# VITA-Group/FasterSeg

Measured on AMD Instinct MI355X. Metric: supernet train-step images/sec @1024x2048 (1/2/4/8 GPU) + student fps, higher is better.
Workload: dtype bf16; 1 GPU; C2 student fps (BASELINE configs[1]): searched arch_1 (eval build, branches 1/32+1/16) inference 1x3x1024x2048, 19 classes, fp32 logits at input resolution; parallelism=replicas x1 (inference does not shard: no collective)

## Files before the change

### fasterseg_amd/_lib.py

```python
import ctypes
import os

_HERE = os.path.dirname(os.path.abspath(__file__))
LIB_PATH = os.path.join(_HERE, "libfasterseg_hip.so")

EXPECTED_ABI = 218
FS_F32, FS_BF16 = 0, 1
FS_CONV_RELU, FS_CONV_TRANSPOSED, FS_CONV_ACCUM, FS_CONV_RELU_TAIL = 1, 2, 4, 8
FS_CONV_KSPLIT, FS_CONV_NO_KSPLIT, FS_CONV_KSPLIT16 = 0x4000, 0x8000, 0x14000

c_int, c_ll, c_float, c_vp = ctypes.c_int, ctypes.c_longlong, ctypes.c_float, ctypes.c_void_p


class ConvDesc(ctypes.Structure):
    _fields_ = [(n, c_int) for n in ("N", "H", "W", "Cin", "Cout", "R", "S", "stride", "pad", "Ho", "Wo",
                                     "x_cs", "y_cs", "dtype", "flags", "w_os", "w_ts", "vr_H", "vr_W", "vr_relu", "bn_groups",
                                     "n_seg", "n_jump", "k_seg", "k_jump", "g_jump")]


class ZoomDesc(ctypes.Structure):
    _fields_ = [(n, c_int) for n in ("N", "H", "W", "Cin", "Cmid", "Cout", "h", "w", "Ho", "Wo", "x_cs", "y_cs", "dtype", "down", "up")]


class LogitsDesc(ctypes.Structure):
    _fields_ = [(n, c_int) for n in ("N", "h", "w", "C", "cs", "H", "W", "dtype")]


class ResizeDesc(ctypes.Structure):
    _fields_ = [(n, c_int) for n in ("N", "Hi", "Wi", "Ho", "Wo", "C", "x_cs", "y_cs", "dtype", "relu", "out_nchw")]


class EvalWindowDesc(ctypes.Structure):
    _fields_ = [(n, c_int) for n in ("H", "W", "rows", "cols", "top", "left", "oy", "ox", "crop_h", "crop_w", "pad_mode", "flip")] + [
        ("mean", c_float * 3), ("std", c_float * 3)]


class TrainSample(ctypes.Structure):
    _fields_ = [(n, c_int) for n in ("H", "W", "mirror", "sh", "sw", "pos_h", "pos_w", "top", "left", "rows", "cols", "ylin", "xlin",
                                     "ynn", "xnn", "reserved")]
# ... 98 lines not shown
    "fs_nchw_to_nhwc": [c_vp, c_int, c_int, c_int, c_int, c_vp, c_vp, c_int, c_int, c_int],
    "fs_nhwc_to_nchw": [c_vp, c_int, c_int, c_int, c_int, c_vp, c_int, c_int, c_vp],
    "fs_copy_channels": [c_vp, c_ll, c_int, c_vp, c_int, c_vp, c_int, c_int],
    "fs_axpy_channels": [c_vp, c_ll, c_int, c_vp, c_int, c_vp, c_vp, c_int, c_int, c_int],
    "fs_dot": [c_vp, c_ll, c_int, c_vp, c_int, c_vp, c_int, c_int, c_vp],
    "fs_weighted_sum": [c_vp, c_ll, c_int, c_int, c_vp, c_vp, c_vp, c_vp, c_int, c_int],
    "fs_weighted_sum_bwd": [c_vp, c_ll, c_int, c_int, c_vp, c_int, c_vp, c_vp, c_vp, c_int],
    "fs_weighted_sum_dots": [c_vp, c_ll, c_int, c_int, c_vp, c_int, c_vp, c_vp, c_int, c_vp],
    "fs_ohem_ce_fwd": [c_vp, c_vp, c_vp, c_ll, c_int, c_ll, c_int, c_vp, c_vp, c_vp],
    "fs_ohem_ce_bwd": [c_vp, c_vp, c_vp, c_vp, c_vp, c_vp, c_ll, c_int, c_ll, c_vp],
    "fs_ohem_ce_bwd_coef": [c_vp, c_vp, c_vp, c_vp, c_vp, c_vp, c_ll, c_int, c_ll, c_vp],
    "fs_ohem_select": [c_vp, c_vp, c_vp, c_vp, c_ll, c_int, c_int, c_vp, c_float, c_ll, c_vp, c_vp, c_vp, c_vp, c_ll],
    "fs_kl_distill_fwd": [c_vp, c_vp, c_vp, c_ll, c_int, c_ll, c_vp, c_vp, c_vp],
    "fs_ohem_ce_up_fwd": [c_vp, ctypes.POINTER(LogitsDesc), c_vp, c_vp, c_int, c_vp, c_vp, c_vp],
    "fs_ohem_ce_up_bwd": [c_vp, ctypes.POINTER(LogitsDesc), c_vp, c_vp, c_vp, c_vp, c_vp, c_vp, c_vp, c_ll],
    "fs_ohem_ce_up_bwd_coef": [c_vp, ctypes.POINTER(LogitsDesc), c_vp, c_vp, c_vp, c_vp, c_vp, c_vp, c_vp, c_ll],
    "fs_kl_distill_up_fwd": [c_vp, ctypes.POINTER(LogitsDesc), c_vp, ctypes.POINTER(LogitsDesc), c_vp, c_vp, c_vp, c_vp],
    "fs_kl_distill_up_bwd": [c_vp, ctypes.POINTER(LogitsDesc), c_vp, ctypes.POINTER(LogitsDesc), c_vp, c_vp, c_vp, c_vp, c_vp, c_vp,
                             c_ll],
    "fs_kl_distill_bwd": [c_vp, c_vp, c_vp, c_vp, c_vp, c_vp, c_ll, c_int, c_ll, c_vp],
    "fs_exec_program": [c_vp, c_vp, c_ll, c_vp, c_vp, c_int],
    "fs_exec_program_streams": [c_vp, c_int, c_vp, c_ll, c_vp, c_vp, c_int],
    "fs_exec_program_group": [c_vp, c_int, c_vp, c_vp, c_vp, c_vp, c_int],
    "fs_sgd_momentum_multi": [c_vp, c_vp, c_vp, c_int, c_vp, c_vp, c_vp, c_vp, c_float, c_float, c_float, c_int, c_int],
    "fs_refresh_weights": [c_vp, c_vp, c_int, c_vp, c_int],
}
_SPECIAL = {
    "fs_last_error": ([], ctypes.c_char_p),
    "fs_version": ([], c_int),
    "fs_struct_size": ([c_int], c_int),
    "fs_packed_weight_elems": ([c_int, c_int, c_int, c_int], c_ll),
    "fs_debug_force_conv_cfg": ([c_int], None),
    "fs_debug_stem_mfma": ([c_int], None),
    "fs_packed_weight_frag_elems": ([c_int, c_int, c_int], c_ll),
    "fs_sgd_chunk_elems": ([], c_int),
    "fs_sgd_tensor_chunks": ([c_ll, c_int, c_int, c_int], c_ll),
    "fs_refresh_chunk_elems": ([], c_int),
    "fs_refresh_entry_chunks": ([ctypes.POINTER(RefreshEntry)], c_ll),
    "fs_loss_up_workspace_bytes": ([ctypes.POINTER(LogitsDesc)], c_ll),
    "fs_ohem_select_workspace_bytes": ([c_ll], c_ll),
    "fs_train_batch_args_bytes": ([c_int], c_ll),
    "fs_zoom_cell_supported": ([ctypes.POINTER(ZoomDesc)], c_int),
    "fs_workspace_counter_bytes": ([], c_ll),
    "fs_set_deterministic": ([c_int], None),
    "fs_get_deterministic": ([], c_int),
    "fs_set_fp32_split": ([c_int], None),
    "fs_get_fp32_split": ([], c_int),
    "fs_census_enable": ([c_int], None),
    "fs_census_read": ([c_vp, c_int], c_int),
    "fs_census_read_kernels": ([c_vp, c_int], c_int),
    "fs_census_tag": ([c_int], None),
    "fs_census_read_tags": ([c_int, c_vp, c_vp], c_int),
    "fs_event_create": ([], c_vp),
    "fs_event_destroy": ([c_vp], None),
}
ALL_SYMBOLS = sorted(list(SIGNATURES) + list(_SPECIAL))

_lib = None


class FasterSegHipError(RuntimeError):
    pass


def lib():
    global _lib
# ... 39 lines not shown
```

### fasterseg_amd/csrc/resize.hip

```cpp
#include "common.h"
#include "group.h"

namespace fs {

static inline float host_scale(int in, int out) { return out > 1 ? (float)(in - 1) / (float)(out - 1) : 0.f; }

struct ResizeArgs {
    int N; DivInt Hi, Wi, Ho, Wo, cv; float rh, rw; const void* a; int a_cs; const void* b; int b_cs; void* out; int out_cs; int relu;
};

template <typename T>
__device__ __forceinline__ void bilinear_fwd_body(const ResizeArgs& q, int bx, int gx) {
    constexpr int VEC = Elem<T>::VEC;
    const int N = q.N, Hi = q.Hi, Wi = q.Wi, Ho = q.Ho, Wo = q.Wo, cv = q.cv, x_cs = q.a_cs, y_cs = q.out_cs, relu = q.relu;
    const float rh = q.rh, rw = q.rw;
    const T* __restrict__ x = (const T*)q.a;
    T* __restrict__ y = (T*)q.out;
    const long long total = (long long)N * Ho * Wo * cv;
    for (long long idx = bx * (long long)blockDim.x + threadIdx.x; idx < total; idx += (long long)gx * blockDim.x) {
        long long t = idx, u = fast_div(t, q.cv);
        const int c = (int)(t - u * cv) * VEC; t = u; u = fast_div(t, q.Wo);
        const int ow = (int)(t - u * Wo); t = u; u = fast_div(t, q.Ho);
        const int oh = (int)(t - u * Ho);
        const int n = (int)u;
        const Tap th = make_tap(rh, oh, Hi), tw = make_tap(rw, ow, Wi);
        const T* base = x + (long long)n * Hi * Wi * x_cs + c;
        float p00[VEC], p01[VEC], p10[VEC], p11[VEC];
        Elem<T>::unpack(ldg16(base + ((long long)th.i0 * Wi + tw.i0) * x_cs), p00);
        Elem<T>::unpack(ldg16(base + ((long long)th.i0 * Wi + tw.i1) * x_cs), p01);
        Elem<T>::unpack(ldg16(base + ((long long)th.i1 * Wi + tw.i0) * x_cs), p10);
        Elem<T>::unpack(ldg16(base + ((long long)th.i1 * Wi + tw.i1) * x_cs), p11);
#pragma unroll
        for (int i = 0; i < VEC; ++i) {
            float o = th.l0 * (tw.l0 * p00[i] + tw.l1 * p01[i]) + th.l1 * (tw.l0 * p10[i] + tw.l1 * p11[i]);
            p00[i] = relu ? fmaxf(o, 0.f) : o;
        }
        stg16(y + (((long long)n * Ho + oh) * Wo + ow) * y_cs + c, Elem<T>::pack(p00));
    }
}

template <typename T> struct Quad;
template <> struct Quad<float> {
    static __device__ __forceinline__ void load(const float* p, float* o) {
        const f32x4 v = *reinterpret_cast<const f32x4*>(p);
        o[0] = v[0]; o[1] = v[1]; o[2] = v[2]; o[3] = v[3];
    }
};
template <> struct Quad<bf16_t> {
    static __device__ __forceinline__ void load(const bf16_t* p, float* o) {
        const uint2 v = *reinterpret_cast<const uint2*>(p);
        o[0] = __uint_as_float(v.x << 16); o[1] = __uint_as_float(v.x & 0xffff0000u);
        o[2] = __uint_as_float(v.y << 16); o[3] = __uint_as_float(v.y & 0xffff0000u);
    }
};
template <typename TO> __device__ __forceinline__ void store4(TO* dst, const float* v);
template <> __device__ __forceinline__ void store4<float>(float* dst, const float* v) {
    __builtin_nontemporal_store(f32x4{v[0], v[1], v[2], v[3]}, reinterpret_cast<f32x4*>(dst));
}
template <> __device__ __forceinline__ void store4<bf16_t>(bf16_t* dst, const float* v) {
    uint2 o;
    o.x = (uint32_t)f32_to_bf16(v[0]) | ((uint32_t)f32_to_bf16(v[1]) << 16);
    o.y = (uint32_t)f32_to_bf16(v[2]) | ((uint32_t)f32_to_bf16(v[3]) << 16);
    *reinterpret_cast<uint2*>(dst) = o;
}

template <typename T, typename TO>
__global__ __launch_bounds__(256) void bilinear_fwd_nchw_kernel(int N, int Hi, int Wi, int Ho, int Wo, int C, float rh, float rw,
                                                                const T* __restrict__ x, int x_cs, TO* __restrict__ y) {
    const int wq = Wo >> 2;
    const int cg = (C + 3) >> 2;
    const long long total = (long long)N * cg * Ho * wq;
    for (long long idx = blockIdx.x * (long long)blockDim.x + threadIdx.x; idx < total;
         idx += (long long)gridDim.x * blockDim.x) {
        long long t = idx;
        const int ow0 = divmod32(t, wq) * 4;
        const int oh = divmod32(t, Ho);
        const int c0 = divmod32(t, cg) * 4;
        const int n = (int)t;
        const Tap th = make_tap(rh, oh, Hi);
        const T* r0 = x + ((long long)n * Hi + th.i0) * Wi * x_cs + c0;
        const T* r1 = x + ((long long)n * Hi + th.i1) * Wi * x_cs + c0;
        float out[4][4];
#pragma unroll
        for (int q = 0; q < 4; ++q) {
            const Tap tw = make_tap(rw, ow0 + q, Wi);
            float p00[4], p01[4], p10[4], p11[4];
            Quad<T>::load(r0 + (long long)tw.i0 * x_cs, p00);
            Quad<T>::load(r0 + (long long)tw.i1 * x_cs, p01);
            Quad<T>::load(r1 + (long long)tw.i0 * x_cs, p10);
            Quad<T>::load(r1 + (long long)tw.i1 * x_cs, p11);
#pragma unroll
            for (int k = 0; k < 4; ++k)
                out[k][q] = th.l0 * (tw.l0 * p00[k] + tw.l1 * p01[k]) + th.l1 * (tw.l0 * p10[k] + tw.l1 * p11[k]);
        }
#pragma unroll
        for (int k = 0; k < 4; ++k)
            if (c0 + k < C) store4<TO>(y + (((long long)n * C + c0 + k) * Ho + oh) * Wo + ow0, out[k]);
    }
}

template <typename T, typename TO>
__global__ void bilinear_fwd_nchw_scalar_kernel(int N, int Hi, int Wi, int Ho, int Wo, int C, float rh, float rw,
                                                const T* __restrict__ x, int x_cs, TO* __restrict__ y) {
    const long long total = (long long)N * C * Ho * Wo;
    for (long long idx = blockIdx.x * (long long)blockDim.x + threadIdx.x; idx < total;
         idx += (long long)gridDim.x * blockDim.x) {
        long long t = idx;
        const int ow = divmod32(t, Wo);
        const int oh = divmod32(t, Ho);
        const int c = divmod32(t, C);
        const int n = (int)t;
        const Tap th = make_tap(rh, oh, Hi), tw = make_tap(rw, ow, Wi);
        const T* b = x + (long long)n * Hi * Wi * x_cs + c;
        const float p00 = Elem<T>::load(b + ((long long)th.i0 * Wi + tw.i0) * x_cs);
        const float p01 = Elem<T>::load(b + ((long long)th.i0 * Wi + tw.i1) * x_cs);
        const float p10 = Elem<T>::load(b + ((long long)th.i1 * Wi + tw.i0) * x_cs);
        const float p11 = Elem<T>::load(b + ((long long)th.i1 * Wi + tw.i1) * x_cs);
        Elem<TO>::store(y + idx, th.l0 * (tw.l0 * p00 + tw.l1 * p01) + th.l1 * (tw.l0 * p10 + tw.l1 * p11));
    }
}

__device__ __forceinline__ void cand_range(float scale, int i, int out_size, int& lo, int& hi) {
    if (scale <= 0.f) {
        lo = 0;
        hi = out_size - 1;
        return;
    }
    const float inv = 1.f / scale;
    lo = (int)floorf((float)(i - 1) * inv) - 1;
    hi = (int)ceilf((float)(i + 1) * inv) + 1;
    if (lo < 0) lo = 0;
    if (hi > out_size - 1) hi = out_size - 1;
}
__device__ __forceinline__ float tap_weight(const Tap& t, int i) {
    float w = 0.f;
    if (t.i0 == i) w += t.l0;
    if (t.i1 == i) w += t.l1;
    return w;
}

constexpr int BWD_TAPS = 6;

template <typename T>
__device__ __forceinline__ void bilinear_bwd_body(const ResizeArgs& q, int bx, int gx) {
    constexpr int VEC = Elem<T>::VEC;
// ... 163 lines not shown
        const int ih = divmod32(t, Hi);
        const int c = divmod32(t, C);
        const int n = (int)t;
        int lo, hi;
        cand_range(rh, ih, Ho, lo, hi);
        const float* plane = tmp + ((long long)n * C + c) * Ho * Wi + iw;
        float acc = 0.f;
        for (int o0 = lo; o0 <= hi; o0 += 8) {
            float v[8];
#pragma unroll
            for (int u = 0; u < 8; ++u) v[u] = plane[(long long)min(o0 + u, Ho - 1) * Wi];
#pragma unroll
            for (int u = 0; u < 8; ++u) {
                const int oh = o0 + u;
                const float w = (oh <= hi) ? tap_weight(make_tap(rh, oh, Hi), ih) : 0.f;
                acc += w * v[u];
            }
        }
        Elem<T>::store(dx + (((long long)n * Hi + ih) * Wi + iw) * dx_cs + c, acc);
    }
}

static inline int grid_for(long long work, int block = 256, int cap = 16384) {
    long long g = (work + block - 1) / block;
    if (g < 1) g = 1;
    if (g > cap) g = cap;
    return (int)g;
}

}

using namespace fs;

static fs_status check_resize(const char* fn, const fs_resize_desc* d) {
    FS_REQUIRE(d, FS_ERR_INVALID, "%s: null descriptor", fn);
    FS_REQUIRE(d->N > 0 && d->Hi > 0 && d->Wi > 0 && d->Ho > 0 && d->Wo > 0 && d->C > 0, FS_ERR_INVALID,
               "%s: non-positive dimension", fn);
    FS_REQUIRE(d->dtype == FS_F32 || d->dtype == FS_BF16, FS_ERR_INVALID, "%s: bad dtype", fn);
    if (!d->out_nchw) {
        const int vec = vec_elems(d->dtype);
        FS_REQUIRE(d->C % vec == 0 && d->x_cs % vec == 0 && d->y_cs % vec == 0 && d->x_cs >= d->C && d->y_cs >= d->C,
                   FS_ERR_UNSUPPORTED, "%s: C=%d / strides (%d,%d) must be multiples of %d", fn, d->C, d->x_cs, d->y_cs, vec);
    } else {
        FS_REQUIRE(d->x_cs >= ((d->C + 3) / 4) * 4 && d->x_cs % 4 == 0, FS_ERR_INVALID,
                   "%s: NCHW output needs the input channel stride padded to a multiple of 4 (got %d for C=%d)", fn, d->x_cs,
                   d->C);
        FS_REQUIRE(!d->relu, FS_ERR_UNSUPPORTED, "%s: relu not supported with NCHW output", fn);
    }
    return FS_OK;
}

extern "C" fs_status fs_bilinear_fwd(void* stream, const fs_resize_desc* d, const void* x, void* y) {
    fs_status s = check_resize("fs_bilinear_fwd", d);
    if (s != FS_OK) return s;
    FS_REQUIRE(x && y, FS_ERR_INVALID, "fs_bilinear_fwd: null pointer");
    const float rh = host_scale(d->Hi, d->Ho), rw = host_scale(d->Wi, d->Wo);
    hipStream_t st = (hipStream_t)stream;
    FS_REQUIRE(aligned16(x) && aligned16(y), FS_ERR_INVALID, "fs_bilinear_fwd: operands must be 16-byte aligned");
    if (!d->out_nchw) {
        const int cv = d->C / vec_elems(d->dtype);
        const long long total = (long long)d->N * d->Ho * d->Wo * cv;
        const ResizeArgs q{d->N, d->Hi, d->Wi, d->Ho, d->Wo, cv, rh, rw, x, d->x_cs, nullptr, 0, y, d->y_cs, d->relu};
        FS_NOTE_BYTES((double)d->N * d->C * elem_size(d->dtype) * ((double)d->Hi * d->Wi + (double)d->Ho * d->Wo));
        if (d->dtype == FS_F32) FS_LAUNCH((bilinear_fwd_kernel<float>), dim3(grid_for(total)), dim3(256), 0, st, q);
        else FS_LAUNCH((bilinear_fwd_kernel<bf16_t>), dim3(grid_for(total)), dim3(256), 0, st, q);
    } else {
        const bool out_f32 = (d->out_nchw == 1) || d->dtype == FS_F32;
        if (d->Wo % 4 == 0) {
            const long long total = (long long)d->N * ((d->C + 3) / 4) * d->Ho * (d->Wo / 4);
            const dim3 g(grid_for(total));
            if (d->dtype == FS_F32)
                FS_LAUNCH((bilinear_fwd_nchw_kernel<float, float>), g, dim3(256), 0, st, d->N, d->Hi, d->Wi, d->Ho, d->Wo,
                                   d->C, rh, rw, (const float*)x, d->x_cs, (float*)y);
            else if (out_f32)
                FS_LAUNCH((bilinear_fwd_nchw_kernel<bf16_t, float>), g, dim3(256), 0, st, d->N, d->Hi, d->Wi, d->Ho, d->Wo,
                                   d->C, rh, rw, (const bf16_t*)x, d->x_cs, (float*)y);
            else
                FS_LAUNCH((bilinear_fwd_nchw_kernel<bf16_t, bf16_t>), g, dim3(256), 0, st, d->N, d->Hi, d->Wi, d->Ho,
                                   d->Wo, d->C, rh, rw, (const bf16_t*)x, d->x_cs, (bf16_t*)y);
        } else {
            const long long total = (long long)d->N * d->C * d->Ho * d->Wo;
            const dim3 g(grid_for(total));
            if (d->dtype == FS_F32)
                FS_LAUNCH((bilinear_fwd_nchw_scalar_kernel<float, float>), g, dim3(256), 0, st, d->N, d->Hi, d->Wi, d->Ho,
                                   d->Wo, d->C, rh, rw, (const float*)x, d->x_cs, (float*)y);
            else if (out_f32)
                FS_LAUNCH((bilinear_fwd_nchw_scalar_kernel<bf16_t, float>), g, dim3(256), 0, st, d->N, d->Hi, d->Wi, d->Ho,
                                   d->Wo, d->C, rh, rw, (const bf16_t*)x, d->x_cs, (float*)y);
            else
                FS_LAUNCH((bilinear_fwd_nchw_scalar_kernel<bf16_t, bf16_t>), g, dim3(256), 0, st, d->N, d->Hi, d->Wi,
                                   d->Ho, d->Wo, d->C, rh, rw, (const bf16_t*)x, d->x_cs, (bf16_t*)y);
        }
    }
    return check_launch("fs_bilinear_fwd");
}

extern "C" fs_status fs_bilinear_bwd_nchw(void* stream, const fs_resize_desc* d, const float* dy, float* workspace, void* dx) {
    fs_status s = check_resize("fs_bilinear_bwd_nchw", d);
    if (s != FS_OK) return s;
    FS_REQUIRE(d->out_nchw == 1, FS_ERR_INVALID, "fs_bilinear_bwd_nchw: descriptor must have out_nchw = 1");
    FS_REQUIRE(dy && workspace && dx, FS_ERR_INVALID, "fs_bilinear_bwd_nchw: null pointer");
// ... 86 lines not shown
```

### fasterseg_amd/csrc/stem.hip

```cpp
#include "common.h"

namespace fs {

template <typename T>
__global__ __launch_bounds__(256) void stem_conv_kernel(int N, int H, int W, int Ho, int Wo, int Cout,
                                                        const float* __restrict__ x, const float* __restrict__ w,
                                                        const float* __restrict__ scale, const float* __restrict__ shift,
                                                        T* __restrict__ y, int y_cs, int relu) {
    const int co0 = blockIdx.y * 16;
    const long long total = (long long)N * Ho * Wo;
    for (long long pix = blockIdx.x * (long long)blockDim.x + threadIdx.x; pix < total;
         pix += (long long)gridDim.x * blockDim.x) {
        const int ow = (int)(pix % Wo);
        const int oh = (int)((pix / Wo) % Ho);
        const int n = (int)(pix / ((long long)Wo * Ho));
        float in[27];
#pragma unroll
        for (int c = 0; c < 3; ++c)
#pragma unroll
            for (int r = 0; r < 3; ++r)
#pragma unroll
                for (int s = 0; s < 3; ++s) {
                    const int ih = oh * 2 - 1 + r, iw = ow * 2 - 1 + s;
                    const bool ok = (unsigned)ih < (unsigned)H && (unsigned)iw < (unsigned)W;
// ... 84 lines not shown
        T* dst = y + pix * y_cs + co0;
        if (co0 + 16 <= Cout) {
#pragma unroll
            for (int v = 0; v < 16 / VEC; ++v) stg16(dst + v * VEC, Elem<T>::pack(out + v * VEC));
        } else {
            for (int k = 0; k < 16 && co0 + k < Cout; ++k) Elem<T>::store(dst + k, out[k]);
        }
    }
}




struct StemTapOff {
    int off[2][2][8];
};

__host__ __device__ constexpr int stem_tap_offset(int k) {
    return k >= 27 ? -1
                   : ((((k / 3) % 3 == 1) ? 0 : 1) * 3 + (k % 3)) * (S_ROWS * S_PITCH) + ((k / 3) / 3) * S_PITCH + (((k / 3) % 3 == 0) ? 1 : 2);
}

__device__ __forceinline__ void split_bf16(const float (&v)[8], u32x4& hi, u32x4& lo) {
#pragma unroll
    for (int i = 0; i < 4; ++i) {
        const float a = v[2 * i], b = v[2 * i + 1];
        const uint32_t h = pack2_bf16(a, b);
        const float ra = a - __uint_as_float(h << 16), rb = b - __uint_as_float(h & 0xffff0000u);
        hi[i] = h;
        lo[i] = pack2_bf16(ra, rb);
    }
}

__global__ __launch_bounds__(256) void stem_mfma_kernel(int H, int W, int Ho, int Wo, int Cout, const float* __restrict__ x,
                                                        const float* __restrict__ w, const float* __restrict__ scale,
                                                        const float* __restrict__ shift, bf16_t* __restrict__ y, int y_cs, int relu) {
    constexpr int WIN = 2 * 3 * S_ROWS * S_PITCH;
    constexpr int OUT_PITCH = 32 * 2 + 16;
    __shared__ __attribute__((aligned(16))) float win[WIN + 4];
    __shared__ __attribute__((aligned(16))) unsigned char sout[4][32 * OUT_PITCH];
    const int tid = threadIdx.x, lane = tid & 63, wave = tid >> 6, l31 = lane & 31, half = lane >> 5;
    const int ow0 = blockIdx.x * S_TW, oh0 = blockIdx.y * S_TH, n = blockIdx.z;
    constexpr int VPR = S_HALF / 2;
    for (int v = tid; v < 3 * S_ROWS * VPR; v += 256) {
        const int c = v / (S_ROWS * VPR);
        const int rem = v - c * (S_ROWS * VPR);
        const int r = rem / VPR, q = rem - r * VPR;
        const int ih = 2 * oh0 - 1 + r, iw = 2 * ow0 - 4 + 4 * q;
        f32x4 t = {0.f, 0.f, 0.f, 0.f};
        if ((unsigned)ih < (unsigned)H && iw >= 0 && iw + 3 < W)
            t = *reinterpret_cast<const f32x4*>(x + (((long long)n * 3 + c) * H + ih) * W + iw);
        float* ev = win + ((0 * 3 + c) * S_ROWS + r) * S_PITCH;
        float* od = win + ((1 * 3 + c) * S_ROWS + r) * S_PITCH;
        ev[2 * q] = t[0]; od[2 * q] = t[1];
        ev[2 * q + 1] = t[2]; od[2 * q + 1] = t[3];
    }
    if (tid < 4) win[WIN + tid] = 0.f;
    const int ntiles = (Cout + 31) / 32;
    u32x4 bh[2][2], bl[2][2];
#pragma unroll
    for (int t = 0; t < 2; ++t)
#pragma unroll
        for (int kk = 0; kk < 2; ++kk) {
            float wv[8];
            const int co = t * 32 + l31;
#pragma unroll
            for (int e = 0; e < 8; ++e) {
                const int k = kk * 16 + half * 8 + e;
                wv[e] = (t < ntiles && co < Cout && k < 27) ? w[co * 27 + k] : 0.f;
            }
            split_bf16(wv, bh[t][kk], bl[t][kk]);
        }
    __syncthreads();
    const int ty = wave;
    const int oh = oh0 + ty;
    unsigned char* so = sout[wave];
#pragma unroll
    for (int h = 0; h < 2; ++h) {
        const int tx = 32 * h + l31;
        const float* base = win + (2 * ty) * S_PITCH + tx;
        u32x4 ah[2], al[2];
#pragma unroll
        for (int kk = 0; kk < 2; ++kk) {
            float av[8];
#pragma unroll
            for (int e = 0; e < 8; ++e) {
                constexpr int dummy = 0;
                (void)dummy;
                const int o0 = stem_tap_offset(kk * 16 + e), o1 = stem_tap_offset(kk * 16 + 8 + e);
                const float* p0 = o0 >= 0 ? base + o0 : win + WIN;
                const float* p1 = o1 >= 0 ? base + o1 : win + WIN;
                av[e] = *(half ? p1 : p0);
            }
            split_bf16(av, ah[kk], al[kk]);
        }
#pragma unroll
        for (int t = 0; t < 2; ++t) {
            if (t >= ntiles) break;
            f32x16 acc;
#pragma unroll
            for (int r = 0; r < 16; ++r) acc[r] = 0.f;
#pragma unroll
            for (int kk = 0; kk < 2; ++kk) {
                acc = __builtin_amdgcn_mfma_f32_32x32x16_bf16(__builtin_bit_cast(bf16x8, al[kk]), __builtin_bit_cast(bf16x8, bh[t][kk]), acc, 0, 0, 0);
                acc = __builtin_amdgcn_mfma_f32_32x32x16_bf16(__builtin_bit_cast(bf16x8, ah[kk]), __builtin_bit_cast(bf16x8, bl[t][kk]), acc, 0, 0, 0);
                acc = __builtin_amdgcn_mfma_f32_32x32x16_bf16(__builtin_bit_cast(bf16x8, ah[kk]), __builtin_bit_cast(bf16x8, bh[t][kk]), acc, 0, 0, 0);
            }
            const int co = t * 32 + l31;
            const bool cvalid = co < Cout;
            const float sc = (scale && cvalid) ? scale[co] : 1.f, sh = (shift && cvalid) ? shift[co] : 0.f;
#pragma unroll
            for (int r = 0; r < 16; ++r) {
                const int prow = (r & 3) + 8 * (r >> 2) + 4 * half;
                float o = acc[r] * sc + sh;
                if (relu) o = fmaxf(o, 0.f);
                *reinterpret_cast<bf16_t*>(so + prow * OUT_PITCH + l31 * 2) = f32_to_bf16(o);
            }
            __builtin_amdgcn_wave_barrier();
            const int cbase = t * 32;
            const int nvalid = Cout - cbase < 32 ? Cout - cbase : 32;
#pragma unroll
            for (int ps = 0; ps < 2; ++ps) {
                const int prow = ps * 16 + (lane >> 2), seg = lane & 3;
                const int ow = ow0 + 32 * h + prow;
                if (oh < Ho && ow < Wo && seg * 8 < nvalid)
                    stg16(y + (((long long)n * Ho + oh) * Wo + ow) * y_cs + cbase + seg * 8,
                          *reinterpret_cast<const u32x4*>(so + prow * OUT_PITCH + seg * 16));
            }
            __builtin_amdgcn_wave_barrier();
        }
    }
}

}

using namespace fs;

static int g_stem_mfma = 1;
extern "C" void fs_debug_stem_mfma(int on) { g_stem_mfma = on; }

extern "C" fs_status fs_conv_stem_fwd(void* stream, int N, int H, int W, int Cout, const float* x, const float* w,
                                      const float* scale, const float* shift, void* y, int y_cs, int dtype, int relu) {
    FS_REQUIRE(x && w && y, FS_ERR_INVALID, "fs_conv_stem_fwd: null pointer");
    FS_REQUIRE(N > 0 && H > 1 && W > 1 && Cout > 0, FS_ERR_INVALID, "fs_conv_stem_fwd: bad shape");
    FS_REQUIRE(dtype == FS_F32 || dtype == FS_BF16, FS_ERR_INVALID, "fs_conv_stem_fwd: bad dtype");
    FS_REQUIRE(y_cs >= Cout && y_cs % vec_elems(dtype) == 0 && aligned16(y), FS_ERR_INVALID,
               "fs_conv_stem_fwd: output slice misaligned (y_cs=%d)", y_cs);
    const int Ho = (H + 2 - 3) / 2 + 1, Wo = (W + 2 - 3) / 2 + 1;
    if (W % 4 == 0 && aligned16(x) && N <= 65535) {
        dim3 tiles((unsigned)((Wo + S_TW - 1) / S_TW), (unsigned)((Ho + S_TH - 1) / S_TH), (unsigned)N);
        if (dtype == FS_BF16 && Cout <= 64 && Cout % 8 == 0 && g_stem_mfma) {
            FS_LAUNCH(stem_mfma_kernel, tiles, dim3(256), 0, (hipStream_t)stream, H, W, Ho, Wo, Cout, x, w, scale, shift,
                               (bf16_t*)y, y_cs, relu);
            return check_launch("fs_conv_stem_fwd");
        }
        if (dtype == FS_F32)
            FS_LAUNCH((stem_lds_kernel<float>), tiles, dim3(256), 0, (hipStream_t)stream, H, W, Ho, Wo, Cout, x, w, scale,
                               shift, (float*)y, y_cs, relu);
        else
            FS_LAUNCH((stem_lds_kernel<bf16_t>), tiles, dim3(256), 0, (hipStream_t)stream, H, W, Ho, Wo, Cout, x, w, scale,
                               shift, (bf16_t*)y, y_cs, relu);
        return check_launch("fs_conv_stem_fwd");
    }
    const long long total = (long long)N * Ho * Wo;
    long long gx = (total + 255) / 256;
    if (gx > 32768) gx = 32768;
    dim3 grid((unsigned)gx, (Cout + 15) / 16);
    if (dtype == FS_F32)
        FS_LAUNCH((stem_conv_kernel<float>), grid, dim3(256), 0, (hipStream_t)stream, N, H, W, Ho, Wo, Cout, x, w, scale,
                           shift, (float*)y, y_cs, relu);
    else
        FS_LAUNCH((stem_conv_kernel<bf16_t>), grid, dim3(256), 0, (hipStream_t)stream, N, H, W, Ho, Wo, Cout, x, w, scale,
                           shift, (bf16_t*)y, y_cs, relu);
    return check_launch("fs_conv_stem_fwd");
}
```

### include/fasterseg_hip.h

```cpp
#ifndef FASTERSEG_HIP_H
#define FASTERSEG_HIP_H

#ifdef __cplusplus
extern "C" {
#endif

typedef enum { FS_OK = 0, FS_ERR_INVALID = 1, FS_ERR_UNSUPPORTED = 2, FS_ERR_LAUNCH = 3 } fs_status;
typedef enum { FS_F32 = 0, FS_BF16 = 1 } fs_dtype;

#define FS_CONV_RELU        1
#define FS_CONV_TRANSPOSED  2
#define FS_CONV_ACCUM       4
#define FS_CONV_RELU_TAIL   8
#define FS_CONV_TILE_32     0x1000
#define FS_CONV_TILE_64     0x2000
#define FS_CONV_TILE_128    0x3000
#define FS_CONV_TILE_MASK   0x3000
#define FS_CONV_KSPLIT      0x4000
#define FS_CONV_NO_KSPLIT   0x8000
#define FS_CONV_KSPLIT16    0x14000

typedef struct fs_conv_desc {
    int N, H, W, Cin;
    int Cout, R, S;
    int stride, pad;
    int Ho, Wo;
    int x_cs, y_cs;
    int dtype;
    int flags;
    int w_os, w_ts;
    int vr_H, vr_W;
    int vr_relu;
    int bn_groups;
    int n_seg, n_jump;
    int k_seg, k_jump;
    int g_jump;
} fs_conv_desc;

typedef struct fs_resize_desc {
    int N, Hi, Wi, Ho, Wo, C;
    int x_cs, y_cs;
    int dtype;
    int relu;
    int out_nchw;
} fs_resize_desc;

const char* fs_last_error(void);
#define FS_ABI_VERSION 218
int fs_version(void);
void fs_set_deterministic(int on);
int fs_get_deterministic(void);
void fs_set_fp32_split(int on);
int fs_get_fp32_split(void);
int fs_struct_size(int which);
void fs_debug_force_conv_cfg(int cfg);
long long fs_packed_weight_elems(int Cout, int R, int S, int Cin);

fs_status fs_pack_weight(void* stream, const float* w_oihw, long long o_stride, long long i_stride,
                         int Cout, int Cin, int R, int S, int dtype, int transpose_flip, void* w_packed);
fs_status fs_unpack_weight_grad(void* stream, const float* dw_packed, int Cout, int Cin, int R, int S,
                                float* dw_oihw, long long o_stride, long long i_stride, int accumulate);

fs_status fs_conv2d_fwd(void* stream, const fs_conv_desc* d, const void* x, const void* w_packed,
                        const float* scale, const float* shift, void* y, float* stats);
#define FS_CONV_WORKSPACE_BYTES (16ll << 20)
fs_status fs_conv2d_fwd_ws(void* stream, const fs_conv_desc* d, const void* x, const void* w_packed,
                           const float* scale, const float* shift, void* y, float* stats, void* workspace,
                           long long workspace_bytes);

fs_status fs_factorized_reduce_fwd(void* stream, const fs_conv_desc* d1, const void* x1, const void* w1_packed, void* y1, float* stats1,
                                   const fs_conv_desc* d2, const void* x2, const void* w2_packed, void* y2, float* stats2);
fs_status fs_factorized_reduce_wgrad(void* stream, const fs_conv_desc* d1, const void* x1, const void* dy1, float* dw1_packed,
                                     const fs_conv_desc* d2, const void* x2, const void* dy2, float* dw2_packed);
fs_status fs_time_op(void* stream, const fs_conv_desc* d, const void* x, const void* w_packed, void* y, int warmup, int iters, float* ms_out);

long long fs_packed_weight_frag_elems(int Cout, int Cin, int dtype);
fs_status fs_pack_weight_frag(void* stream, const float* w_oihw, long long o_stride, long long i_stride, int Cout, int Cin,
                              int dtype, void* w_frag);
fs_status fs_conv3x3_s1_fwd(void* stream, const fs_conv_desc* d, const void* x, const void* w_frag, const float* scale,
                            const float* shift, void* y, float* stats);
fs_status fs_conv3x3_halo_plan(const fs_conv_desc* d, int has_stats, int* tile, int* ksplit, long long* workgroups);

typedef struct fs_zoom_desc {
    int N, H, W, Cin;
    int Cmid, Cout;
    int h, w;
    int Ho, Wo;
    int x_cs, y_cs;
    int dtype;
    int down, up;
} fs_zoom_desc;
int fs_zoom_cell_supported(const fs_zoom_desc* d);
fs_status fs_zoom_cell_fwd(void* stream, const fs_zoom_desc* d, const void* x, const void* w1_frag, const float* scale1,
                           const float* shift1, const void* w2_frag, const float* scale2, const float* shift2, void* y);

fs_status fs_conv2d_wgrad(void* stream, const fs_conv_desc* d, const void* x, const void* dy, float* dw_packed);
fs_status fs_conv2d_wgrad_strided(void* stream, const fs_conv_desc* d, const void* x, const void* dy, float* dw,
                                  long long o_stride, long long i_stride, long long t_stride);
#define FS_WS_COUNTER_BYTES 65536
long long fs_workspace_counter_bytes(void);
fs_status fs_conv2d_wgrad_ws(void* stream, const fs_conv_desc* d, const void* x, const void* dy, float* dw, long long o_stride,
                             long long i_stride, long long t_stride, void* workspace, long long workspace_bytes);

fs_status fs_conv_stem_fwd(void* stream, int N, int H, int W, int Cout, const float* x_nchw, const float* w_packed,
                           const float* scale, const float* shift, void* y, int y_cs, int dtype, int relu);

void fs_debug_stem_mfma(int on);

fs_status fs_bilinear_fwd(void* stream, const fs_resize_desc* d, const void* x, void* y);
fs_status fs_bilinear_bwd(void* stream, const fs_resize_desc* d, const void* dy, const void* y_out, void* dx);
fs_status fs_bilinear_bwd_nchw(void* stream, const fs_resize_desc* d, const float* dy, float* workspace, void* dx);

fs_status fs_bn_finalize(void* stream, int C, long long count, const float* stats, const float* gamma,
                         const float* beta, float eps, float momentum, float* running_mean, float* running_var,
                         float* mean, float* invstd, float* scale, float* shift, long long* num_batches_tracked);
fs_status fs_bn_train_apply(void* stream, long long pixels, int C, const void* x, int x_cs, const float* stats,
                            const float* gamma, const float* beta, float eps, float momentum, float* running_mean,
                            float* running_var, long long* num_batches_tracked, float* saved, void* y, int y_cs, int dtype,
                            int relu);
fs_status fs_affine_act(void* stream, long long pixels, int C, const void* x, int x_cs, const float* scale,
                        const float* shift, void* y, int y_cs, int dtype, int relu);
fs_status fs_channel_stats(void* stream, long long pixels, int C, const void* x, int x_cs, int dtype, float* stats);
fs_status fs_bn_group_fwd(void* stream, long long pixels, int C, int groups, void* z, int z_cs, const float* partials, int splits,
                          const float* gamma, const float* beta, float eps, float momentum, float* running_mean,
                          float* running_var, long long* num_batches_tracked, float* saved, void* y, int y_cs, int dtype, int relu);
fs_status fs_bn_group_bwd(void* stream, long long pixels, int C, int groups, const void* z, int z_cs, const void* dy, int dy_cs,
                          const void* y_out, int y_cs, const float* saved, const float* gamma, int dtype, int relu, void* dz,
                          int dz_cs, float* red, float* dgamma_acc, float* dbeta_acc);
fs_status fs_bn_bwd_reduce(void* stream, long long pixels, int C, const void* x, int x_cs, const void* dy, int dy_cs,
                           const void* y_out, int y_cs, const float* mean, const float* invstd, int dtype, int relu,
                           float* red);
fs_status fs_bn_bwd_apply(void* stream, long long pixels, int C, const void* x, int x_cs, const void* dy, int dy_cs,
                          const void* y_out, int y_cs, const float* mean, const float* invstd, const float* gamma,
                          const float* red, long long count, int dtype, int relu, void* dx, int dx_cs,
                          float* dgamma_acc, float* dbeta_acc);
fs_status fs_channel_stats_g(void* stream, long long pixels, int C, int groups, const void* x, int x_cs, int dtype, float* stats);
fs_status fs_channel_stats_ws(void* stream, long long pixels, int C, int groups, const void* x, int x_cs, int dtype, float* stats,
                              void* workspace, long long workspace_bytes);
fs_status fs_bn_bwd_reduce_ws(void* stream, long long pixels, int C, int groups, const void* x, int x_cs, const void* dy, int dy_cs,
                              const void* y_out, int y_cs, const float* mean, const float* invstd, int saved_stride, int dtype,
                              int relu, float* red, void* workspace, long long workspace_bytes);
fs_status fs_bn_train_apply_g(void* stream, long long pixels, int C, int groups, const void* x, int x_cs, const float* stats,
// ... 259 lines not shown
```

Measured before the change: 3063 frames/s.

## Tile logits bilinear upsample through LDS and make stem conv persistent with prefetch

Adds a tiled NCHW bilinear upsample kernel that stages the input window for a 32x256 output tile in LDS. It reuses horizontally interpolated rows across consecutive output rows, replacing four scattered global loads per output quad; the kernel is enabled by default. The stem MFMA conv becomes a persistent kernel sized to the CU count, double-buffering the input window in LDS and prefetching the next tile's loads into registers while computing the current one. The tap computation also changes to a contract-off variant, which may alter rounding slightly.

```diff
diff --git a/fasterseg_amd/_lib.py b/fasterseg_amd/_lib.py
--- a/fasterseg_amd/_lib.py
+++ b/fasterseg_amd/_lib.py
@@ -4,7 +4,7 @@
 _HERE = os.path.dirname(os.path.abspath(__file__))
 LIB_PATH = os.path.join(_HERE, "libfasterseg_hip.so")
 
-EXPECTED_ABI = 218
+EXPECTED_ABI = 219
 FS_F32, FS_BF16 = 0, 1
 FS_CONV_RELU, FS_CONV_TRANSPOSED, FS_CONV_ACCUM, FS_CONV_RELU_TAIL = 1, 2, 4, 8
 FS_CONV_KSPLIT, FS_CONV_NO_KSPLIT, FS_CONV_KSPLIT16 = 0x4000, 0x8000, 0x14000
@@ -169,6 +169,8 @@
     "fs_packed_weight_elems": ([c_int, c_int, c_int, c_int], c_ll),
     "fs_debug_force_conv_cfg": ([c_int], None),
     "fs_debug_stem_mfma": ([c_int], None),
+    "fs_debug_stem_blocks": ([c_int], None),
+    "fs_debug_logits_tiled": ([c_int], None),
     "fs_packed_weight_frag_elems": ([c_int, c_int, c_int], c_ll),
     "fs_sgd_chunk_elems": ([], c_int),
     "fs_sgd_tensor_chunks": ([c_ll, c_int, c_int, c_int], c_ll),
diff --git a/fasterseg_amd/csrc/resize.hip b/fasterseg_amd/csrc/resize.hip
--- a/fasterseg_amd/csrc/resize.hip
+++ b/fasterseg_amd/csrc/resize.hip
@@ -39,6 +39,17 @@
     }
 }
 
+__device__ __forceinline__ Tap make_tap_rn(float scale, int dst, int in_size) {
+#pragma clang fp contract(off)
+    Tap t;
+    const float src = scale * (float)dst;
+    t.i0 = (int)src;
+    t.i1 = t.i0 + ((t.i0 < in_size - 1) ? 1 : 0);
+    t.l1 = src - (float)t.i0;
+    t.l0 = 1.f - t.l1;
+    return t;
+}
+
 template <typename T> struct Quad;
 template <> struct Quad<float> {
     static __device__ __forceinline__ void load(const float* p, float* o) {
@@ -77,13 +88,13 @@
         const int oh = divmod32(t, Ho);
         const int c0 = divmod32(t, cg) * 4;
         const int n = (int)t;
-        const Tap th = make_tap(rh, oh, Hi);
+        const Tap th = make_tap_rn(rh, oh, Hi);
         const T* r0 = x + ((long long)n * Hi + th.i0) * Wi * x_cs + c0;
         const T* r1 = x + ((long long)n * Hi + th.i1) * Wi * x_cs + c0;
         float out[4][4];
 #pragma unroll
         for (int q = 0; q < 4; ++q) {
-            const Tap tw = make_tap(rw, ow0 + q, Wi);
+            const Tap tw = make_tap_rn(rw, ow0 + q, Wi);
             float p00[4], p01[4], p10[4], p11[4];
             Quad<T>::load(r0 + (long long)tw.i0 * x_cs, p00);
             Quad<T>::load(r0 + (long long)tw.i1 * x_cs, p01);
@@ -96,6 +107,68 @@
 #pragma unroll
         for (int k = 0; k < 4; ++k)
             if (c0 + k < C) store4<TO>(y + (((long long)n * C + c0 + k) * Ho + oh) * Wo + ow0, out[k]);
+    }
+}
+
+constexpr int LT_TR = 32, LT_TW = 256, LT_SEG = 8;
+constexpr int LT_LDS_BYTES = 64 * 1024;
+static inline int lt_span(int t, float r) { return (int)((float)(t - 1) * r) + 4; }
+
+template <typename T, typename TO>
+__global__ __launch_bounds__(256) void bilinear_fwd_nchw_tiled_kernel(int Hi, int Wi, int Ho, int Wo, int C, float rh, float rw,
+                                                                      const T* __restrict__ x, int x_cs, TO* __restrict__ y) {
+    extern __shared__ __attribute__((aligned(16))) float lt_win[];
+    const int tid = threadIdx.x, lane = tid & 63, wave = tid >> 6;
+    const int ow_t = blockIdx.x * LT_TW, oh_t = blockIdx.y * LT_TR, n = blockIdx.z;
+    const int rows = min(LT_TR, Ho - oh_t), cols = min(LT_TW, Wo - ow_t);
+    const int r_lo = make_tap_rn(rh, oh_t, Hi).i0, c_lo = make_tap_rn(rw, ow_t, Wi).i0;
+    const int nr = make_tap_rn(rh, oh_t + rows - 1, Hi).i1 - r_lo + 1, nc = make_tap_rn(rw, ow_t + cols - 1, Wi).i1 - c_lo + 1;
+    const int plane = nr * nc;
+    const int cg = (C + 3) >> 2;
+    const T* src = x + (long long)n * Hi * Wi * x_cs;
+    for (int it = tid; it < cg * plane; it += 256) {
+        const int g = it / plane, p = it - g * plane;
+        const int r = p / nc, c = p - r * nc;
+        float v[4];
+        Quad<T>::load(src + ((long long)(r_lo + r) * Wi + c_lo + c) * x_cs + g * 4, v);
+#pragma unroll
+        for (int k = 0; k < 4; ++k) lt_win[(g * 4 + k) * plane + p] = v[k];
+    }
+    __syncthreads();
+    const int ow0 = ow_t + lane * 4;
+    if (ow0 >= Wo) return;
+    Tap tw[4];
+    int o0[4], o1[4];
+#pragma unroll
+    for (int q = 0; q < 4; ++q) {
+        tw[q] = make_tap_rn(rw, ow0 + q, Wi);
+        o0[q] = tw[q].i0 - c_lo;
+        o1[q] = tw[q].i1 - c_lo;
+    }
+    const int nseg = (rows + LT_SEG - 1) / LT_SEG;
+    for (int it = wave; it < C * nseg; it += 4) {
+        const int c = it / nseg, r0 = (it - c * nseg) * LT_SEG, r1 = min(r0 + LT_SEG, rows);
+        const float* pl = lt_win + c * plane;
+        TO* dst = y + (((long long)n * C + c) * Ho + oh_t + r0) * Wo + ow0;
+        int cur = -1;
+        float h0[4] = {0.f, 0.f, 0.f, 0.f}, h1[4] = {0.f, 0.f, 0.f, 0.f};
+        for (int r = r0; r < r1; ++r, dst += Wo) {
+            const Tap th = make_tap_rn(rh, oh_t + r, Hi);
+            if (th.i0 != cur) {
+                cur = th.i0;
+                const float* a = pl + (th.i0 - r_lo) * nc;
+                const float* b = pl + (th.i1 - r_lo) * nc;
+#pragma unroll
+                for (int q = 0; q < 4; ++q) {
+                    h0[q] = tw[q].l0 * a[o0[q]] + tw[q].l1 * a[o1[q]];
+                    h1[q] = tw[q].l0 * b[o0[q]] + tw[q].l1 * b[o1[q]];
+                }
+            }
+            float o[4];
+#pragma unroll
+            for (int q = 0; q < 4; ++q) o[q] = th.l0 * h0[q] + th.l1 * h1[q];
+            store4<TO>(dst, o);
+        }
     }
 }
 
@@ -110,7 +183,7 @@
         const int oh = divmod32(t, Ho);
         const int c = divmod32(t, C);
         const int n = (int)t;
-        const Tap th = make_tap(rh, oh, Hi), tw = make_tap(rw, ow, Wi);
+        const Tap th = make_tap_rn(rh, oh, Hi), tw = make_tap_rn(rw, ow, Wi);
         const T* b = x + (long long)n * Hi * Wi * x_cs + c;
         const float p00 = Elem<T>::load(b + ((long long)th.i0 * Wi + tw.i0) * x_cs);
         const float p01 = Elem<T>::load(b + ((long long)th.i0 * Wi + tw.i1) * x_cs);
@@ -340,6 +413,9 @@
 
 using namespace fs;
 
+static int g_logits_tiled = 1;
+extern "C" void fs_debug_logits_tiled(int on) { g_logits_tiled = on; }
+
 static fs_status check_resize(const char* fn, const fs_resize_desc* d) {
     FS_REQUIRE(d, FS_ERR_INVALID, "%s: null descriptor", fn);
     FS_REQUIRE(d->N > 0 && d->Hi > 0 && d->Wi > 0 && d->Ho > 0 && d->Wo > 0 && d->C > 0, FS_ERR_INVALID,
@@ -374,7 +450,21 @@
         else FS_LAUNCH((bilinear_fwd_kernel<bf16_t>), dim3(grid_for(total)), dim3(256), 0, st, q);
     } else {
         const bool out_f32 = (d->out_nchw == 1) || d->dtype == FS_F32;
-        if (d->Wo % 4 == 0) {
+        const long long lt_bytes = (long long)((d->C + 3) / 4) * 16 * lt_span(LT_TR, rh) * lt_span(LT_TW, rw);
+        if (d->Wo % 4 == 0 && g_logits_tiled && lt_bytes <= LT_LDS_BYTES && d->N <= 65535 && d->Ho <= 65535 * LT_TR && d->Hi < 32768 &&
+            d->Wi < 32768) {
+            const dim3 g((unsigned)((d->Wo + LT_TW - 1) / LT_TW), (unsigned)((d->Ho + LT_TR - 1) / LT_TR), (unsigned)d->N);
+            const size_t lds = (size_t)lt_bytes;
+            if (d->dtype == FS_F32)
+                FS_LAUNCH((bilinear_fwd_nchw_tiled_kernel<float, float>), g, dim3(256), lds, st, d->Hi, d->Wi, d->Ho, d->Wo, d->C, rh, rw,
+                                   (const float*)x, d->x_cs, (float*)y);
+            else if (out_f32)
+                FS_LAUNCH((bilinear_fwd_nchw_tiled_kernel<bf16_t, float>), g, dim3(256), lds, st, d->Hi, d->Wi, d->Ho, d->Wo, d->C, rh, rw,
+                                   (const bf16_t*)x, d->x_cs, (float*)y);
+            else
+                FS_LAUNCH((bilinear_fwd_nchw_tiled_kernel<bf16_t, bf16_t>), g, dim3(256), lds, st, d->Hi, d->Wi, d->Ho, d->Wo, d->C, rh,
+                                   rw, (const bf16_t*)x, d->x_cs, (bf16_t*)y);
+        } else if (d->Wo % 4 == 0) {
             const long long total = (long long)d->N * ((d->C + 3) / 4) * d->Ho * (d->Wo / 4);
             const dim3 g(grid_for(total));
             if (d->dtype == FS_F32)
diff --git a/fasterseg_amd/csrc/stem.hip b/fasterseg_amd/csrc/stem.hip
--- a/fasterseg_amd/csrc/stem.hip
+++ b/fasterseg_amd/csrc/stem.hip
@@ -140,103 +140,152 @@
     }
 }
 
-__global__ __launch_bounds__(256) void stem_mfma_kernel(int H, int W, int Ho, int Wo, int Cout, const float* __restrict__ x,
+constexpr int S_VPR = S_HALF / 2;
+constexpr int S_VECS = 3 * S_ROWS * S_VPR;
+constexpr int S_LD = (S_VECS + 255) / 256;
+constexpr int S_WIN = 2 * 3 * S_ROWS * S_PITCH;
+
+__device__ __forceinline__ void stem_tile_origin(int t, int tyn, int txn, int& n, int& oh0, int& ow0) {
+    const int u = t / tyn;
+    n = u / txn;
+    oh0 = (t - u * tyn) * S_TH;
+    ow0 = (u - n * txn) * S_TW;
+}
+
+__device__ __forceinline__ void stem_load_window(f32x4 (&reg)[S_LD], const float* __restrict__ x, int H, int W, int n, int oh0, int ow0,
+                                                 int tid) {
+#pragma unroll
+    for (int j = 0; j < S_LD; ++j) {
+        const int v = tid + 256 * j;
+        const int c = v / (S_ROWS * S_VPR);
+        const int rem = v - c * (S_ROWS * S_VPR);
+        const int r = rem / S_VPR, q = rem - r * S_VPR;
+        const int ih = 2 * oh0 - 1 + r, iw = 2 * ow0 - 4 + 4 * q;
+        f32x4 t = {0.f, 0.f, 0.f, 0.f};
+        if (v < S_VECS && (unsigned)ih < (unsigned)H && iw >= 0 && iw + 3 < W)
+            t = *reinterpret_cast<const f32x4*>(x + (((long long)n * 3 + c) * H + ih) * W + iw);
+        reg[j] = t;
+    }
+}
+
+__device__ __forceinline__ void stem_write_window(const f32x4 (&reg)[S_LD], float* win, int tid) {
+#pragma unroll
+    for (int j = 0; j < S_LD; ++j) {
+        const int v = tid + 256 * j;
+        if (v < S_VECS) {
+            const int c = v / (S_ROWS * S_VPR);
+            const int rem = v - c * (S_ROWS * S_VPR);
+            const int r = rem / S_VPR, q = rem - r * S_VPR;
+            float* ev = win + ((0 * 3 + c) * S_ROWS + r) * S_PITCH;
+            float* od = win + ((1 * 3 + c) * S_ROWS + r) * S_PITCH;
+            ev[2 * q] = reg[j][0]; od[2 * q] = reg[j][1];
+            ev[2 * q + 1] = reg[j][2]; od[2 * q + 1] = reg[j][3];
+        }
+    }
+}
+
+template <int NT>
+__global__ __launch_bounds__(256, NT == 1 ? 4 : 3) void stem_mfma_kernel(int N, int H, int W, int Ho, int Wo, int Cout, const float* __restrict__ x,
                                                         const float* __restrict__ w, const float* __restrict__ scale,
                                                         const float* __restrict__ shift, bf16_t* __restrict__ y, int y_cs, int relu) {
-    constexpr int WIN = 2 * 3 * S_ROWS * S_PITCH;
     constexpr int OUT_PITCH = 32 * 2 + 16;
-    __shared__ __attribute__((aligned(16))) float win[WIN + 4];
+    __shared__ __attribute__((aligned(16))) float win[2][S_WIN + 4];
     __shared__ __attribute__((aligned(16))) unsigned char sout[4][32 * OUT_PITCH];
     const int tid = threadIdx.x, lane = tid & 63, wave = tid >> 6, l31 = lane & 31, half = lane >> 5;
-    const int ow0 = blockIdx.x * S_TW, oh0 = blockIdx.y * S_TH, n = blockIdx.z;
-    constexpr int VPR = S_HALF / 2;
-    for (int v = tid; v < 3 * S_ROWS * VPR; v += 256) {
-        const int c = v / (S_ROWS * VPR);
-        const int rem = v - c * (S_ROWS * VPR);
-        const int r = rem / VPR, q = rem - r * VPR;
-        const int ih = 2 * oh0 - 1 + r, iw = 2 * ow0 - 4 + 4 * q;
-        f32x4 t = {0.f, 0.f, 0.f, 0.f};
-        if ((unsigned)ih < (unsigned)H && iw >= 0 && iw + 3 < W)
-            t = *reinterpret_cast<const f32x4*>(x + (((long long)n * 3 + c) * H + ih) * W + iw);
-        float* ev = win + ((0 * 3 + c) * S_ROWS + r) * S_PITCH;
-        float* od = win + ((1 * 3 + c) * S_ROWS + r) * S_PITCH;
-        ev[2 * q] = t[0]; od[2 * q] = t[1];
-        ev[2 * q + 1] = t[2]; od[2 * q + 1] = t[3];
-    }
-    if (tid < 4) win[WIN + tid] = 0.f;
-    const int ntiles = (Cout + 31) / 32;
-    u32x4 bh[2][2], bl[2][2];
-#pragma unroll
-    for (int t = 0; t < 2; ++t)
+    const int txn = (Wo + S_TW - 1) / S_TW, tyn = (Ho + S_TH - 1) / S_TH;
+    const int total = N * txn * tyn;
+    int t = blockIdx.x;
+    if (t >= total) return;
+    int n, oh0, ow0;
+    f32x4 reg[S_LD];
+    stem_tile_origin(t, tyn, txn, n, oh0, ow0);
+    stem_load_window(reg, x, H, W, n, oh0, ow0, tid);
+    if (tid < 4) win[0][S_WIN + tid] = 0.f;
+    else if (tid < 8) win[1][S_WIN + tid - 4] = 0.f;
+    u32x4 bh[NT][2], bl[NT][2];
+#pragma unroll
+    for (int nt = 0; nt < NT; ++nt)
 #pragma unroll
         for (int kk = 0; kk < 2; ++kk) {
             float wv[8];
-            const int co = t * 32 + l31;
+            const int co = nt * 32 + l31;
 #pragma unroll
             for (int e = 0; e < 8; ++e) {
                 const int k = kk * 16 + half * 8 + e;
-                wv[e] = (t < ntiles && co < Cout && k < 27) ? w[co * 27 + k] : 0.f;
-            }
-            split_bf16(wv, bh[t][kk], bl[t][kk]);
-        }
+                wv[e] = (co < Cout && k < 27) ? w[co * 27 + k] : 0.f;
+            }
+            split_bf16(wv, bh[nt][kk], bl[nt][kk]);
+        }
+    stem_write_window(reg, win[0], tid);
     __syncthreads();
     const int ty = wave;
-    const int oh = oh0 + ty;
     unsigned char* so = sout[wave];
-#pragma unroll
-    for (int h = 0; h < 2; ++h) {
-        const int tx = 32 * h + l31;
-        const float* base = win + (2 * ty) * S_PITCH + tx;
-        u32x4 ah[2], al[2];
-#pragma unroll
-        for (int kk = 0; kk < 2; ++kk) {
-            float av[8];
-#pragma unroll
-            for (int e = 0; e < 8; ++e) {
-                constexpr int dummy = 0;
-                (void)dummy;
-                const int o0 = stem_tap_offset(kk * 16 + e), o1 = stem_tap_offset(kk * 16 + 8 + e);
-                const float* p0 = o0 >= 0 ? base + o0 : win + WIN;
-                const float* p1 = o1 >= 0 ? base + o1 : win + WIN;
-                av[e] = *(half ? p1 : p0);
-            }
-            split_bf16(av, ah[kk], al[kk]);
-        }
-#pragma unroll
-        for (int t = 0; t < 2; ++t) {
-            if (t >= ntiles) break;
-            f32x16 acc;
-#pragma unroll
-            for (int r = 0; r < 16; ++r) acc[r] = 0.f;
+    for (int buf = 0;; buf ^= 1) {
+        const int tn = t + (int)gridDim.x;
+        const bool more = tn < total;
+        int nn = 0, noh0 = 0, now0 = 0;
+        if (more) {
+            stem_tile_origin(tn, tyn, txn, nn, noh0, now0);
+            stem_load_window(reg, x, H, W, nn, noh0, now0, tid);
+        }
+        const float* wb = win[buf];
+        const int oh = oh0 + ty;
+#pragma unroll 1
+        for (int h = 0; h < 2; ++h) {
+            const int tx = 32 * h + l31;
+            const float* base = wb + (2 * ty) * S_PITCH + tx;
+            u32x4 ah[2], al[2];
 #pragma unroll
             for (int kk = 0; kk < 2; ++kk) {
-                acc = __builtin_amdgcn_mfma_f32_32x32x16_bf16(__builtin_bit_cast(bf16x8, al[kk]), __builtin_bit_cast(bf16x8, bh[t][kk]), acc, 0, 0, 0);
-                acc = __builtin_amdgcn_mfma_f32_32x32x16_bf16(__builtin_bit_cast(bf16x8, ah[kk]), __builtin_bit_cast(bf16x8, bl[t][kk]), acc, 0, 0, 0);
-                acc = __builtin_amdgcn_mfma_f32_32x32x16_bf16(__builtin_bit_cast(bf16x8, ah[kk]), __builtin_bit_cast(bf16x8, bh[t][kk]), acc, 0, 0, 0);
-            }
-            const int co = t * 32 + l31;
-            const bool cvalid = co < Cout;
-            const float sc = (scale && cvalid) ? scale[co] : 1.f, sh = (shift && cvalid) ? shift[co] : 0.f;
-#pragma unroll
-            for (int r = 0; r < 16; ++r) {
-                const int prow = (r & 3) + 8 * (r >> 2) + 4 * half;
-                float o = acc[r] * sc + sh;
-                if (relu) o = fmaxf(o, 0.f);
-                *reinterpret_cast<bf16_t*>(so + prow * OUT_PITCH + l31 * 2) = f32_to_bf16(o);
-            }
-            __builtin_amdgcn_wave_barrier();
-            const int cbase = t * 32;
-            const int nvalid = Cout - cbase < 32 ? Cout - cbase : 32;
-#pragma unroll
-            for (int ps = 0; ps < 2; ++ps) {
-                const int prow = ps * 16 + (lane >> 2), seg = lane & 3;
-                const int ow = ow0 + 32 * h + prow;
-                if (oh < Ho && ow < Wo && seg * 8 < nvalid)
-                    stg16(y + (((long long)n * Ho + oh) * Wo + ow) * y_cs + cbase + seg * 8,
-                          *reinterpret_cast<const u32x4*>(so + prow * OUT_PITCH + seg * 16));
-            }
-            __builtin_amdgcn_wave_barrier();
-        }
+                float av[8];
+#pragma unroll
+                for (int e = 0; e < 8; ++e) {
+                    const int o0 = stem_tap_offset(kk * 16 + e), o1 = stem_tap_offset(kk * 16 + 8 + e);
+                    const float* p0 = o0 >= 0 ? base + o0 : wb + S_WIN;
+                    const float* p1 = o1 >= 0 ? base + o1 : wb + S_WIN;
+                    av[e] = *(half ? p1 : p0);
+                }
+                split_bf16(av, ah[kk], al[kk]);
+            }
+#pragma unroll
+            for (int nt = 0; nt < NT; ++nt) {
+                f32x16 acc;
+#pragma unroll
+                for (int r = 0; r < 16; ++r) acc[r] = 0.f;
+#pragma unroll
+                for (int kk = 0; kk < 2; ++kk) {
+                    acc = __builtin_amdgcn_mfma_f32_32x32x16_bf16(__builtin_bit_cast(bf16x8, al[kk]), __builtin_bit_cast(bf16x8, bh[nt][kk]), acc, 0, 0, 0);
+                    acc = __builtin_amdgcn_mfma_f32_32x32x16_bf16(__builtin_bit_cast(bf16x8, ah[kk]), __builtin_bit_cast(bf16x8, bl[nt][kk]), acc, 0, 0, 0);
+                    acc = __builtin_amdgcn_mfma_f32_32x32x16_bf16(__builtin_bit_cast(bf16x8, ah[kk]), __builtin_bit_cast(bf16x8, bh[nt][kk]), acc, 0, 0, 0);
+                }
+                const int co = nt * 32 + l31;
+                const bool cvalid = co < Cout;
+                const float sc = (scale && cvalid) ? scale[co] : 1.f, sh = (shift && cvalid) ? shift[co] : 0.f;
+#pragma unroll
+                for (int r = 0; r < 16; ++r) {
+                    const int prow = (r & 3) + 8 * (r >> 2) + 4 * half;
+                    float o = acc[r] * sc + sh;
+                    if (relu) o = fmaxf(o, 0.f);
+                    *reinterpret_cast<bf16_t*>(so + prow * OUT_PITCH + l31 * 2) = f32_to_bf16(o);
+                }
+                __builtin_amdgcn_wave_barrier();
+                const int cbase = nt * 32;
+                const int nvalid = Cout - cbase < 32 ? Cout - cbase : 32;
+#pragma unroll
+                for (int ps = 0; ps < 2; ++ps) {
+                    const int prow = ps * 16 + (lane >> 2), seg = lane & 3;
+                    const int ow = ow0 + 32 * h + prow;
+                    if (oh < Ho && ow < Wo && seg * 8 < nvalid)
+                        stg16(y + (((long long)n * Ho + oh) * Wo + ow) * y_cs + cbase + seg * 8,
+                              *reinterpret_cast<const u32x4*>(so + prow * OUT_PITCH + seg * 16));
+                }
+                __builtin_amdgcn_wave_barrier();
+            }
+        }
+        if (!more) break;
+        stem_write_window(reg, win[buf ^ 1], tid);
+        __syncthreads();
+        t = tn; n = nn; oh0 = noh0; ow0 = now0;
     }
 }
 
@@ -246,6 +295,17 @@
 
 static int g_stem_mfma = 1;
 extern "C" void fs_debug_stem_mfma(int on) { g_stem_mfma = on; }
+static int g_stem_blocks = 0;
+static int compute_units() {
+    static int cus = 0;
+    if (!cus) {
+        int dev = 0, v = 0;
+        if (hipGetDevice(&dev) == hipSuccess && hipDeviceGetAttribute(&v, hipDeviceAttributeMultiprocessorCount, dev) == hipSuccess && v > 0) cus = v;
+        else cus = 256;
+    }
+    return cus;
+}
+extern "C" void fs_debug_stem_blocks(int n) { g_stem_blocks = n; }
 
 extern "C" fs_status fs_conv_stem_fwd(void* stream, int N, int H, int W, int Cout, const float* x, const float* w,
                                       const float* scale, const float* shift, void* y, int y_cs, int dtype, int relu) {
@@ -257,9 +317,16 @@
     const int Ho = (H + 2 - 3) / 2 + 1, Wo = (W + 2 - 3) / 2 + 1;
     if (W % 4 == 0 && aligned16(x) && N <= 65535) {
         dim3 tiles((unsigned)((Wo + S_TW - 1) / S_TW), (unsigned)((Ho + S_TH - 1) / S_TH), (unsigned)N);
-        if (dtype == FS_BF16 && Cout <= 64 && Cout % 8 == 0 && g_stem_mfma) {
-            FS_LAUNCH(stem_mfma_kernel, tiles, dim3(256), 0, (hipStream_t)stream, H, W, Ho, Wo, Cout, x, w, scale, shift,
-                               (bf16_t*)y, y_cs, relu);
+        const long long ntile = (long long)tiles.x * tiles.y * tiles.z;
+        if (dtype == FS_BF16 && Cout <= 64 && Cout % 8 == 0 && g_stem_mfma && ntile < (1ll << 31)) {
+            long long blocks = g_stem_blocks > 0 ? g_stem_blocks : (long long)(Cout <= 32 ? 4 : 3) * compute_units();
+            if (blocks > ntile) blocks = ntile;
+            if (Cout <= 32)
+                FS_LAUNCH(stem_mfma_kernel<1>, dim3((unsigned)blocks), dim3(256), 0, (hipStream_t)stream, N, H, W, Ho, Wo, Cout, x, w,
+                                   scale, shift, (bf16_t*)y, y_cs, relu);
+            else
+                FS_LAUNCH(stem_mfma_kernel<2>, dim3((unsigned)blocks), dim3(256), 0, (hipStream_t)stream, N, H, W, Ho, Wo, Cout, x, w,
+                                   scale, shift, (bf16_t*)y, y_cs, relu);
             return check_launch("fs_conv_stem_fwd");
         }
         if (dtype == FS_F32)
diff --git a/include/fasterseg_hip.h b/include/fasterseg_hip.h
--- a/include/fasterseg_hip.h
+++ b/include/fasterseg_hip.h
@@ -46,7 +46,7 @@
 } fs_resize_desc;
 
 const char* fs_last_error(void);
-#define FS_ABI_VERSION 218
+#define FS_ABI_VERSION 219
 int fs_version(void);
 void fs_set_deterministic(int on);
 int fs_get_deterministic(void);
@@ -106,8 +106,10 @@
                            const float* scale, const float* shift, void* y, int y_cs, int dtype, int relu);
 
 void fs_debug_stem_mfma(int on);
+void fs_debug_stem_blocks(int n);
 
 fs_status fs_bilinear_fwd(void* stream, const fs_resize_desc* d, const void* x, void* y);
+void fs_debug_logits_tiled(int on);
 fs_status fs_bilinear_bwd(void* stream, const fs_resize_desc* d, const void* dy, const void* y_out, void* dx);
 fs_status fs_bilinear_bwd_nchw(void* stream, const fs_resize_desc* d, const float* dy, float* workspace, void* dx);
 
```

Result: faster. 3177 frames/s, median of 6 (+3.7%).
